# cliangyu/video-diffusion

Measured on AMD Instinct MI355X. Metric: denoise-steps/sec, higher is better.
Workload: dtype f32

## Files before the change

include/vd_amd.h:

```cpp
#ifndef VD_AMD_H
#define VD_AMD_H
#ifdef __cplusplus
extern "C" {
#endif

typedef struct vd_config {
    int image_size;
    int num_channels;
    int num_res_blocks;
    int num_heads;
    int T;
    int n_attention_ds;
    int attention_ds[8];
    int use_scale_shift_norm;
    int use_spatial_encoding;
    int use_frame_encoding;
    int enforce_position_invariance;
    int use_rpe_net;
    int allow_interactions_between_padding;
    float rp_alpha, rp_beta, rp_gamma;
    int time_embed_mult;
    int cond_emb_type;
    int learn_sigma;
} vd_config;
// ... 119 lines not shown
int vd_profile_classes(void);
const char* vd_profile_class_name(int i);

int vd_math_mode(void);
long long vd_split_image_u16(long long n_out, long long k_total);

int vd_op_conv(const float* src0, const float* src1, int C0, int Cin, int nfr, int Hs, int Ws, int ups, int stride,
               int pad, int ksz, const float* w_packed, const float* w_frag, const float* w_wino, const float* bias,
               const float* affA, const float* affB, int act, const float* res, const float* fbias, int fbias_ld,
               float* out, int Cout, void* stream);
int vd_conv_stats_split(int Hout);
int vd_conv_wino_block_couts(int nfr, int H, int Cin, int Cout);
int vd_op_conv_stats(const float* src0, int Cin, int nfr, int Hs, int Ws, int ups, const float* w_wino, const float* bias,
                     const float* res, const float* fbias, int fbias_ld, float* out, int Cout, double* gn_part,
                     void* stream);
int vd_op_gn_affine(const double* part0, int split0, int C0, const double* part1, int split1, int C, int nfr, int HW,
                    const float* gamma, const float* beta, const float* film, int film_ld, float* affA, float* affB,
                    void* stream);
int vd_pack_conv3_wino(const float* host_oihw, float* host_out, int O, int I);
int vd_pack_linear_frag(const float* host_w, float* host_out, int N, int K);
int vd_pack_linear_split(const float* host_w, unsigned short* host_out, int N, int K);
int vd_pack_conv3_split(const float* host_oihw, unsigned short* host_out, int O, int I);
int vd_op_conv_split(const float* src0, int Cin, int nfr, int Hs, int Ws, int stride, const void* w_split, const float* bias,
                     const float* res, float* out, int Cout, void* stream);
int vd_pack_conv3_wino_split(const float* host_oihw, unsigned short* host_out, int O, int I);
int vd_op_conv_wino_split(const float* src0, int Cin, int nfr, int Hs, int Ws, int ups, const void* w_split, const float* bias,
                          const float* res, const float* fbias, int fbias_ld, float* out, int Cout, double* gn_part,
                          void* stream);
int vd_op_conv_wino_act(const float* src0, const float* src1, int C0, int Cin, int nfr, int Hs, int Ws, const void* w_split, const float* bias,
                        const float* affA, const float* affB, const float* res, float* out, int Cout, double* gn_part, void* stream);
int vd_conv_wino_act_ok(int nfr, int H, int Cin, int Cout);
int vd_pack_conv3_wino_ups(const float* host_oihw, unsigned short* host_out, int O, int I);
int vd_conv_ups_stats_split(int Hs);
int vd_op_conv_wino_ups(const float* src0, int Cin, int nfr, int Hs, const void* w_ups, const float* bias, float* out, int Cout,
                        double* gn_part, void* stream);
int vd_op_linear_split(const float* a, int M, int K, const void* w_split, const float* bias, const float* res, int act,
                       float* out, int N, void* stream);
int vd_op_linear_split_stats(const float* a, int M, int K, const void* w_split, const float* bias, const float* res, int act,
                             float* out, int N, int HW, double* gn_part, void* stream);
int vd_linear_stats_split(int M, int N, int HW);
int vd_op_gn_fold(const float* src0, const float* src1, int C0, int C, int nfr, int HW, const float* gamma,
                  const float* beta, const float* film, int film_ld, float* affA, float* affB, void* stream);
int vd_op_affine_apply(const float* x, const float* affA, const float* affB, int nfr, int HW, int C, float* y,
                       void* stream);
int vd_op_affine_act(const float* src0, const float* src1, int C0, int C, const float* affA, const float* affB, int nfr,
                     int HW, int act, float* y, void* stream);
int vd_op_gn_temporal(const float* x, const float* gamma, const float* beta, int B, int T, int HW, int C, float* y,
                      void* stream);
int vd_op_attn_spatial(const float* qkv, int nfr, int L, int C, int heads, float* out, void* stream);
int vd_op_attn_temporal(const float* qkv, const float* Rk, const float* Rq, const float* Rv, const float* mask, int B,
                        int T, int HW, int C, int heads, int allow_pad, float* out, void* stream);
int vd_op_out_conv(const float* x, const float* affA, const float* affB, const float* w_packed, const float* bias,
                   int nfr, int H, int W, int C, int Cout, float* out_nchw, void* stream);
int vd_op_gn_bwd(const float* x0, const float* x1, int C0, int C, const float* affA, const float* affB, const float* mr,
                 const float* dy, int act, int nfr, int HW, const float* extra, float* dx0, int acc0, float* dx1, int acc1,
                 void* stream);
int vd_op_gn_temporal_bwd(const float* x, const float* gamma, const float* dy, int B, int T, int HW, int C, int accumulate,
                          float* dx, void* stream);
int vd_op_attn_temporal_bwd(const float* qkv, const float* Rk, const float* Rq, const float* Rv, const float* mask, int B,
                            int T, int HW, int C, int heads, int allow_pad, const float* dout, float* dqkv, void* stream);
int vd_op_attn_spatial_bwd(const float* qkv, int nfr, int L, int C, int heads, const float* dout, float* dqkv, void* stream);
int vd_op_out_conv_bwd(const float* deps, const float* w, int nfr, int H, int W, int C, int Cout, float* da, void* stream);
int vd_op_stem_col2im(const float* dcols, const float* obs, const float* lat, const float* km, int nfr, int H, int W,
                      int cond_mode, float* dx, void* stream);

typedef struct vd_lpips vd_lpips;
int vd_lpips_create(vd_lpips** out);
void vd_lpips_destroy(vd_lpips* h);
int vd_lpips_load_weight(vd_lpips* h, const char* name, const float* host, long long bytes);
long long vd_lpips_dim(int H, int W);
int vd_lpips_embed(vd_lpips* h, int N, int H, int W, const float* frames, float* out, void* stream);
int vd_fps_select(int B, int n_cand, long long D, const float* embs, int n, const int* always_host, int n_always, float* work,
                  int* out, void* stream);

int vd_frame_metrics(int N, int C, int H, int W, const float* gt, const void* pred, int pred_is_u8, double ssim_data_range,
                     double* ssim_out, double* psnr_out, void* stream);
int vd_pair_sqdist(int N, long long D, const float* a, const float* b, double* out, void* stream);

typedef struct vd_i3d vd_i3d;
int vd_i3d_create(vd_i3d** out);
void vd_i3d_destroy(vd_i3d* h);
int vd_i3d_load_weight(vd_i3d* h, const char* name, const float* host, long long bytes);
int vd_i3d_max_frames(void);
int vd_i3d_embed(vd_i3d* h, int N, int T, int H, int W, const unsigned char* videos, float* out, void* stream);
int vd_op_conv3d_same(const float* x, const float* w, const float* bias, int T, int H, int W, int Cin, int Cout, int kt, int kh,
                      int kw, int st, int sh, int sw, int relu, float* out, long long out_stride, void* stream);
int vd_op_maxpool3d_same(const float* x, int T, int H, int W, int C, int kt, int kh, int kw, int st, int sh, int sw, float* out,
                         void* stream);
int vd_op_resize_bilinear_tf1(const unsigned char* frames, int T, int H, int W, float* out, void* stream);

#ifdef __cplusplus
}
#endif
#endif
```

video-diffusion_amd/_lib.py:

```python
import ctypes
import os
import subprocess

_HERE = os.path.dirname(os.path.abspath(__file__))
_CSRC = os.path.join(_HERE, "csrc")
SO_PATH = os.path.join(_HERE, "libvdamd.so")
SOURCES = ["igemm.hip", "conv_wino.hip", "conv_wino_r64.hip", "conv_wino_z128.hip", "gemm_frag.hip", "gemm_split.hip", "split_pack.hip", "norm.hip", "backward.hip", "attn_spatial.hip", "attn_temporal.hip", "attn_temporal_long.hip", "misc.hip", "engine.hip", "lpips.hip", "metrics.hip", "i3d.hip"]
HEADER = os.path.join(os.path.dirname(_HERE), "include", "vd_amd.h")
HEADERS = [os.path.join(_CSRC, "vd_common.h"), os.path.join(_CSRC, "wino_common.h"), HEADER]
SOURCE_FLAGS = {"conv_wino_z128.hip": ["-mllvm", "-pragma-unroll-threshold=1000000"]}


def _toolchain():
    hipcc = os.environ.get("HIPCC", "/opt/rocm/bin/hipcc")
    flags = ["--offload-arch=gfx950", "-O3", "-std=c++17", "-fPIC", "-Wno-unused-value"] + \
        os.environ.get("VD_HIPCC_FLAGS", "").split()
    return hipcc, flags


def _sha(*parts):
    import hashlib
    h = hashlib.sha1()
    for p in parts:
        h.update(p if isinstance(p, bytes) else str(p).encode())
        h.update(b"\0")
    return h.hexdigest()


def _read(path):
    with open(path, "rb") as f:
        return f.read()


def source_sha():
    hipcc, flags = _toolchain()
    return _sha("\0".join(flags), repr(sorted(SOURCE_FLAGS.items())), *[_read(os.path.join(_CSRC, s)) for s in SOURCES], *[_read(h) for h in HEADERS])[:16]


def _stale():
    if not os.path.exists(SO_PATH):
        return True
    try:
        with open(SO_PATH + ".flags") as f:
            return f.read().strip() != source_sha()
    except OSError:
        return True


def build(force=False, verbose=False):
    if not force and not _stale():
        return SO_PATH
    import fcntl
    from concurrent.futures import ThreadPoolExecutor
    with open(SO_PATH + ".lock", "w") as lock:
        fcntl.flock(lock, fcntl.LOCK_EX)
        try:
            if not force and not _stale():
                return SO_PATH
            hipcc, flags = _toolchain()
            sha = source_sha()
            objdir = os.path.join(_CSRC, ".obj")
            os.makedirs(objdir, exist_ok=True)
# ... 90 lines not shown
    "vd_window_generation": (_U, [_P]),
    "vd_set_window_prefix_cache": (_I, [_P, _I]),
    "vd_window_prefix_frames": (_I, [_P]),
    "vd_set_window_suffix_skip": (_I, [_P, _I]),
    "vd_window_suffix_frames": (_I, [_P]),
    "vd_window_begin": (_I, [_P, _I, _I, _P, _P, _P, _P, _P, _P, _I, _I, _I, _F, _U, _U, _L, _P]),
    "vd_window_run": (_I, [_P, _I, _P]),
    "vd_window_graphs": (_I, [_P]),
    "vd_posterior_update": (_I, [_P, _I, _I, _L, _P, _P, _P, _I, _F, _P, _U, _U, _P, _P, _P]),
    "vd_posterior_from_xstart": (_I, [_P, _I, _I, _L, _P, _P, _P, _I, _F, _P, _U, _U, _P, _P, _P, _P]),
    "vd_attn_blocks": (_I, [_P]),
    "vd_attn_block_info": (_I, [_P, _I, ctypes.POINTER(_I), ctypes.POINTER(_I)]),
    "vd_set_attn_capture": (_I, [_P, _P, _P, _I]),
    "vd_bwd_weights_bytes": (_L, [_P]),
    "vd_set_bwd_weight_storage": (_I, [_P, _P, _L, _I]),
    "vd_load_weight_bwd": (_I, [_P, ctypes.c_char_p, _P, _L]),
    "vd_guided_step": (_I, [_P, _I, _I, _P, _P, _P, _P, _P, _P, _I, _P, _P, _P, _P, _P, _P, _P, _P]),
    "vd_q_sample": (_I, [_P, _I, _L, _P, _P, _P, _P, _P]),
    "vd_randn": (_I, [_P, _L, _U, _U, _P]),
    "vd_profile_begin": (_I, []),
    "vd_profile_end": (_I, [_P, _I]),
    "vd_profile_classes": (_I, []),
    "vd_profile_class_name": (ctypes.c_char_p, [_I]),
    "vd_op_conv": (_I, [_P, _P, _I, _I, _I, _I, _I, _I, _I, _I, _I, _P, _P, _P, _P, _P, _P, _I, _P, _P, _I, _P, _I, _P]),
    "vd_conv_stats_split": (_I, [_I]),
    "vd_conv_wino_block_couts": (_I, [_I, _I, _I, _I]),
    "vd_op_conv_stats": (_I, [_P, _I, _I, _I, _I, _I, _P, _P, _P, _P, _I, _P, _I, _P, _P]),
    "vd_op_gn_affine": (_I, [_P, _I, _I, _P, _I, _I, _I, _I, _P, _P, _P, _I, _P, _P, _P]),
    "vd_pack_conv3_wino": (_I, [_P, _P, _I, _I]),
    "vd_pack_linear_frag": (_I, [_P, _P, _I, _I]),
    "vd_pack_linear_split": (_I, [_P, _P, _I, _I]),
    "vd_pack_conv3_wino_split": (_I, [_P, _P, _I, _I]),
    "vd_set_model_mean_type": (_I, [_P, _I]),
    "vd_math_mode": (_I, []),
    "vd_split_image_u16": (_L, [_L, _L]),
    "vd_pack_conv3_wino_ups": (_I, [_P, _P, _I, _I]),
    "vd_conv_ups_stats_split": (_I, [_I]),
    "vd_op_conv_wino_ups": (_I, [_P, _I, _I, _I, _P, _P, _P, _I, _P, _P]),
    "vd_op_conv_wino_split": (_I, [_P, _I, _I, _I, _I, _I, _P, _P, _P, _P, _I, _P, _I, _P, _P]),
    "vd_op_conv_wino_act": (_I, [_P, _P, _I, _I, _I, _I, _I, _P, _P, _P, _P, _P, _P, _I, _P, _P]),
    "vd_conv_wino_act_ok": (_I, [_I, _I, _I, _I]),
    "vd_pack_conv3_split": (_I, [_P, _P, _I, _I]),
    "vd_op_conv_split": (_I, [_P, _I, _I, _I, _I, _I, _P, _P, _P, _P, _I, _P]),
    "vd_op_linear_split": (_I, [_P, _I, _I, _P, _P, _P, _I, _P, _I, _P]),
    "vd_op_linear_split_stats": (_I, [_P, _I, _I, _P, _P, _P, _I, _P, _I, _I, _P, _P]),
    "vd_linear_stats_split": (_I, [_I, _I, _I]),
    "vd_op_gn_fold": (_I, [_P, _P, _I, _I, _I, _I, _P, _P, _P, _I, _P, _P, _P]),
    "vd_op_affine_apply": (_I, [_P, _P, _P, _I, _I, _I, _P, _P]),
    "vd_op_affine_act": (_I, [_P, _P, _I, _I, _P, _P, _I, _I, _I, _P, _P]),
    "vd_op_gn_temporal": (_I, [_P, _P, _P, _I, _I, _I, _I, _P, _P]),
    "vd_op_attn_spatial": (_I, [_P, _I, _I, _I, _I, _P, _P]),
    "vd_op_attn_temporal": (_I, [_P, _P, _P, _P, _P, _I, _I, _I, _I, _I, _I, _P, _P]),
    "vd_op_out_conv": (_I, [_P, _P, _P, _P, _P, _I, _I, _I, _I, _I, _P, _P]),
    "vd_op_gn_bwd": (_I, [_P, _P, _I, _I, _P, _P, _P, _P, _I, _I, _I, _P, _P, _I, _P, _I, _P]),
    "vd_op_gn_temporal_bwd": (_I, [_P, _P, _P, _I, _I, _I, _I, _I, _P, _P]),
    "vd_op_attn_temporal_bwd": (_I, [_P, _P, _P, _P, _P, _I, _I, _I, _I, _I, _I, _P, _P, _P]),
    "vd_op_attn_spatial_bwd": (_I, [_P, _I, _I, _I, _I, _P, _P, _P]),
    "vd_op_out_conv_bwd": (_I, [_P, _P, _I, _I, _I, _I, _I, _P, _P]),
    "vd_op_stem_col2im": (_I, [_P, _P, _P, _P, _I, _I, _I, _I, _P, _P]),
    "vd_lpips_create": (_I, [ctypes.POINTER(_P)]),
    "vd_lpips_destroy": (None, [_P]),
    "vd_lpips_load_weight": (_I, [_P, ctypes.c_char_p, _P, _L]),
    "vd_lpips_dim": (_L, [_I, _I]),
    "vd_lpips_embed": (_I, [_P, _I, _I, _I, _P, _P, _P]),
    "vd_fps_select": (_I, [_I, _I, _L, _P, _I, _P, _I, _P, _P, _P]),
    "vd_frame_metrics": (_I, [_I, _I, _I, _I, _P, _P, _I, _D, _P, _P, _P]),
    "vd_pair_sqdist": (_I, [_I, _L, _P, _P, _P, _P]),
    "vd_i3d_create": (_I, [ctypes.POINTER(_P)]),
    "vd_i3d_destroy": (None, [_P]),
    "vd_i3d_load_weight": (_I, [_P, ctypes.c_char_p, _P, _L]),
    "vd_i3d_max_frames": (_I, []),
    "vd_i3d_embed": (_I, [_P, _I, _I, _I, _I, _P, _P, _P]),
    "vd_op_conv3d_same": (_I, [_P, _P, _P, _I, _I, _I, _I, _I, _I, _I, _I, _I, _I, _I, _I, _P, _L, _P]),
    "vd_op_maxpool3d_same": (_I, [_P, _I, _I, _I, _I, _I, _I, _I, _I, _I, _I, _P, _P]),
    "vd_op_resize_bilinear_tf1": (_I, [_P, _I, _I, _I, _P, _P]),
}

_lib = None


def lib():
    global _lib
    if _lib is None:
        path = os.environ.get("VD_LIB")
        if not path:
            build()
            path = SO_PATH
        L = ctypes.CDLL(path)
        for name, (res, args) in SIGNATURES.items():
            fn = getattr(L, name)
            fn.restype = res
            fn.argtypes = args
        if not os.environ.get("VD_LIB") and L.vd_source_sha().decode() != source_sha():
            raise RuntimeError(f"libvdamd.so was built from other sources ({L.vd_source_sha().decode()}) than the ones beside it "
                               f"({source_sha()}): rebuild (video_diffusion_amd._lib.build(force=True))")
        _lib = L
    return _lib


class VdError(RuntimeError):
    pass


def check(rc):
    if rc != 0:
        msg = lib().vd_last_error().decode(errors="replace")
# ... 15 lines not shown
```

video-diffusion_amd/csrc/engine.hip:

```cpp
#include <cmath>
#include <cstring>
#include <unordered_map>
#include <vector>

#include "../../include/vd_amd.h"
#include "vd_common.h"

namespace vd {

thread_local std::string g_last_error;
void set_error(const std::string& msg) { g_last_error = msg; }

int launch_frame_t(const int64_t* fidx, int B, int T, int center, float* tv, hipStream_t s);

enum ParamKind { PK_RAW = 0, PK_CONV3, PK_STEM, PK_POSENC, PK_OUTCONV, PK_LINF, PK_CONV3W, PK_CONV3S,
                 PK_CONV3WU };

struct Param {
    std::string name;
    int nd = 0;
    long long shape[4] = {1, 1, 1, 1};
    size_t numel = 0;
    size_t packed = 0;
    size_t off = 0;
    int kind = PK_RAW;
    bool loaded = false;
    int frag_rows = 0, frag_row0 = 0;
    int kind_bwd = -1;
    size_t off_bwd = 0, packed_bwd = 0;
};

struct ResP {
    int cin, cout;
    int gn1w, gn1b, c1w, c1b, embw, embb, gn2w, gn2b, c2w, c2b, skw = -1, skb = -1;
    int film_off = 0;
};
struct RpeP { int dw = -1, db = -1, tw = -1, tb = -1, ow = -1, ob = -1, table = -1; int te_off = 0; };
struct AttP { int normw, normb, qkvw, qkvb, projw, projb; };
struct AttnP { int C; AttP sp, tp; RpeP rq, rk, rv; };
struct ConvP { int w, b, c; };
struct Layer { int type; int idx; };
struct Tens { float* p; int C, H; double* part = nullptr; int split = 0; };

struct TapeRes { int idx; Tens x0, x1; bool has_x1; int N; float *A1, *B1, *mr1, *h, *A2, *B2, *mr2, *o; };
struct TapeAttn { int idx; Tens x; int B, T; float *xn, *qkv, *Rk, *Rq, *Rv, *o, *xt, *A, *Bf, *mr, *xn2, *qkv2, *o2, *xs; const float* amask; };
struct TapeConv { int type, idx; Tens in, out; };
struct TapePos { Tens in, out; };
struct TapeOp { int kind, i; };
struct Tape {
    std::vector<TapeOp> ops;
    std::vector<TapeRes> res; std::vector<TapeAttn> attn; std::vector<TapeConv> conv; std::vector<TapePos> pos;
    Tens head; float *headA = nullptr, *headB = nullptr, *head_mr = nullptr;
    void clear() { ops.clear(); res.clear(); attn.clear(); conv.clear(); pos.clear(); }
};

static const int CH_MULT_256[] = {1, 1, 2, 2, 4, 4};
static const int CH_MULT_128[] = {1, 1, 2, 3, 4};
static const int CH_MULT_64[] = {1, 2, 3, 4};
// ... 976 lines not shown
            hs.push_back(h);
        }
        if ((int)i + 1 == n_before_attn && (cfg.use_spatial_encoding || cfg.use_frame_encoding)) {
            const size_t n = (size_t)N * h.H * h.H * h.C;
            float* y = ar.get<float>(n);
            if (!ar.dry) {
                VD_REQUIRE(h.H == pos_res && h.C == pos_ch, "positional encoding shape");
                if ((rc = launch_posenc_add(h.p, cfg.use_spatial_encoding ? W(p_posenc) : nullptr, femb, N, h.H * h.H, h.C, y, st)))
                    return rc;
            }
            if (tape) { tape->ops.push_back(TapeOp{5, (int)tape->pos.size()}); tape->pos.push_back(TapePos{h, Tens{y, h.C, h.H}}); }
            h = Tens{y, h.C, h.H};
        }
    }
    if ((rc = run(middle, h, nullptr, &h))) return rc;
    const int Nsuf = sp ? sp->n : N;
    bool compact = false;
    auto gather_t = [&](const Tens& t) -> Tens {
        const size_t per = (size_t)t.H * t.H * t.C;
        Tens c{ar.get<float>((size_t)Nsuf * per), t.C, t.H, nullptr, t.split};
        if (t.part) c.part = ar.get<double>((size_t)Nsuf * t.split * t.C * 2);
        if (!ar.dry) {
            if (launch_gather_rows(t.p, sp->list, Nsuf, per, c.p, st)) return Tens{};
            if (t.part && launch_gather_rows(reinterpret_cast<const float*>(t.part), sp->list, Nsuf, (size_t)t.split * t.C * 4,
                                             reinterpret_cast<float*>(c.part), st)) return Tens{};
        }
        return c;
    };
    auto go_compact = [&]() -> int {
        float* fc = ar.get<float>((size_t)Nsuf * film_total);
        if (!ar.dry && (rc = launch_gather_rows(film_full, sp->list, Nsuf, film_total, fc, st))) return rc;
        h = gather_t(h);
        VD_REQUIRE(ar.dry || h.p, "suffix skip: gather");
        film = fc; Nrun = Nsuf; g_sel_nfr = N; compact = true;
        return 0;
    };
    if (sp && suf_blk < 0 && (rc = go_compact())) return rc;
    for (size_t i = 0; i < output_blocks.size(); ++i) {
        Tens skip = hs.back(); hs.pop_back();
        if (sp && !compact && (int)i == suf_blk) {
            if ((rc = run(output_blocks[i], h, &skip, &h, 0, suf_layer + 1))) return rc;
            if ((rc = go_compact())) return rc;
            if ((rc = run(output_blocks[i], h, nullptr, &h, suf_layer + 1))) return rc;
            continue;
        }
        if (compact) { skip = gather_t(skip); VD_REQUIRE(ar.dry || skip.p, "suffix skip: gather"); }
        if ((rc = run(output_blocks[i], h, &skip, &h))) return rc;
    }
    float *A, *Bf, *mrh = nullptr;
    if ((rc = gn_fold(h, nullptr, Nrun, p_outgw, p_outgb, nullptr, 0, st, ar, &A, &Bf, &mrh))) return rc;
    if (tape) { tape->head = h; tape->headA = A; tape->headB = Bf; tape->head_mr = mrh; }
    const int oc = cfg.learn_sigma ? 6 : 3;
    float* eps_c = compact ? ar.get<float>((size_t)Nsuf * oc * S * S) : nullptr;
    float* head_t = ar.get<float>((size_t)Nrun * S * S * out_t_cols(oc));
    if (!ar.dry) {
        VD_REQUIRE(h.H == S && h.C == final_ch, "output head shape");
        {
          ProfScope ps(PC_OUT_CONV, 2.0 * Nrun * S * S * h.C * 27.0, 4.0 * Nrun * S * S * (h.C + 3.0), st);
          if (head_gemm_supported(S * S, h.C, out_t_cols(oc))) {
              rc = launch_head_gemm(h.p, A, Bf, W(p_outw) + (size_t)9 * oc * h.C, Nrun, S * S, h.C, out_t_cols(oc), head_t, st);
          } else {
              IgemmArgs g = conv_args(h, nullptr, Nrun, 1, 1, 0);
              g.w = W(p_outw) + (size_t)9 * oc * h.C; g.wsplit = 0; g.affA = A; g.affB = Bf; g.act = 1;
              g.out = head_t; g.ldo = out_t_cols(oc); g.Cout = out_t_cols(oc);
              rc = launch_igemm(g, st);
          }
          if (!rc) rc = launch_out_gather(head_t, W(p_outb), Nrun, S, S, out_t_cols(oc), oc, compact ? eps_c : in.eps, st); }
        if (rc) return rc;
        if (compact) {
            VD_HIP(hipMemsetAsync(in.eps, 0, (size_t)N * oc * S * S * sizeof(float), st));
            if ((rc = launch_scatter_rows(eps_c, sp->list, Nsuf, (size_t)oc * S * S, in.eps, st))) return rc;
        }
    }
    VD_REQUIRE(!ar.overflow, "workspace overflow: the forward asked for more than the dry run measured (this step's output is invalid)");
    return 0;
}

int vd_engine::ensure_ws(int B, int T, bool suffix_plan) {
    const bool suf = suffix_skip_on || suffix_plan;
    if (B == ws_B && T == ws_T && ws && ws_suf == suf) return 0;
    const long long key = ((long long)B << 32) | (unsigned)T | (suf ? 1ll << 61 : 0);
    size_t tail = 0;
    int rc = grow_ws(key, step_tail_bytes(B, T), [&](size_t* peak) {
        Arena dry; dry.dry = true;
        FwdIn fi{}; fi.B = B; fi.T = T;
        int frc = forward(fi, nullptr, dry);
        if (!frc && suf) {
            Arena dry2; dry2.dry = true;
            SuffixPlan wp; wp.n = B * T;
            frc = forward(fi, nullptr, dry2, nullptr, &wp);
            dry.peak = std::max(dry.peak, dry2.peak);
        }
        *peak = dry.peak;
        return frc;
    }, &tail);
    if (rc) return rc;
    ws_B = B; ws_T = T; ws_tail = tail; ws_suf = suf;
    return 0;
}


namespace {
struct GradMap {
    std::unordered_map<const float*, std::pair<float*, bool>> m;
    Arena* ar;
    float* get(const Tens& t, int N, bool* fresh) {
        auto it = m.find(t.p);
        if (it == m.end()) it = m.emplace(t.p, std::make_pair(ar->get<float>((size_t)N * t.H * t.H * t.C), false)).first;
        *fresh = !it->second.second;
        it->second.second = true;
        return it->second.first;
    }
    float* have(const float* p) const { auto it = m.find(p); return it == m.end() ? nullptr : it->second.first; }
};
}

int vd_engine::bwd_linear(const float* dy, int M, int pw, const float* resid, float* out, hipStream_t st) {
    const Param& p = params[pw];
    const int Kb = (int)p.shape[0], Nb = p.kind == PK_STEM ? STEM_KPAD : (int)p.shape[1];
    IgemmArgs g = linear_args(M, Kb, Nb);
// ... 1119 lines not shown
    g.stats = gn_part; g.stats_split = conv_wino_stats_split(g.Ho);
    VD_REQUIRE(conv_wino_supported(g), "vd_op_conv_stats: shape not covered by the Winograd kernel");
    return launch_igemm(g, static_cast<hipStream_t>(stream));
}

int vd_op_gn_affine(const double* part0, int split0, int C0, const double* part1, int split1, int C, int nfr, int HW,
                    const float* gamma, const float* beta, const float* film, int film_ld, float* affA, float* affB,
                    void* stream) {
    return launch_gn_affine(part0, split0, C0, part1, split1, (double)HW * (C / 32), gamma, beta, film, film_ld, nfr, C, affA,
                            affB, static_cast<hipStream_t>(stream));
}

int vd_op_gn_fold(const float* src0, const float* src1, int C0, int C, int nfr, int HW, const float* gamma,
                  const float* beta, const float* film, int film_ld, float* affA, float* affB, void* stream) {
    OpScratch ws(stream);
    const int split = gn_stats_split(nfr, HW, C);
    double* part;
    int rc = ws.get(&part, (size_t)nfr * split * C * 2);
    if (!rc) rc = launch_gn_stats(src0, src1, C0, C, nfr, HW, part, split, ws.st);
    if (!rc) rc = launch_gn_affine(part, split, C, nullptr, 0, (double)HW * (C / 32), gamma, beta, film, film_ld, nfr, C, affA, affB, ws.st);
    return rc;
}

int vd_op_affine_act(const float* src0, const float* src1, int C0, int C, const float* affA, const float* affB, int nfr,
                     int HW, int act, float* y, void* stream) {
    return launch_affine_act(src0, src1, C0, C, affA, affB, nfr, HW, act, y, static_cast<hipStream_t>(stream));
}

int vd_op_affine_apply(const float* x, const float* affA, const float* affB, int nfr, int HW, int C, float* y, void* stream) {
    return launch_affine_apply(x, affA, affB, nfr, HW, C, y, static_cast<hipStream_t>(stream));
}

int vd_op_gn_temporal(const float* x, const float* gamma, const float* beta, int B, int T, int HW, int C, float* y,
                      void* stream) {
    return launch_gn_temporal(x, gamma, beta, B, T, HW, C, y, static_cast<hipStream_t>(stream));
}

int vd_op_attn_spatial(const float* qkv, int nfr, int L, int C, int heads, float* out, void* stream) {
    AttnSpatialArgs a{qkv, out, nfr, L, C, heads, 1.0f / sqrtf((float)(C / heads))};
    return launch_attn_spatial(a, static_cast<hipStream_t>(stream));
}

int vd_op_attn_temporal(const float* qkv, const float* Rk, const float* Rq, const float* Rv, const float* mask, int B,
                        int T, int HW, int C, int heads, int allow_pad, float* out, void* stream) {
    AttnTemporalArgs a{qkv, Rk, Rq, Rv, mask, out, B, T, HW, C, heads, allow_pad, 1.0f / sqrtf((float)(C / heads))};
    return launch_attn_temporal(a, static_cast<hipStream_t>(stream));
}

int vd_op_out_conv(const float* x, const float* affA, const float* affB, const float* w, const float* bias, int nfr,
                   int H, int W, int C, int Cout, float* out, void* stream) {
    return launch_out_conv(x, affA, affB, w, bias, nfr, H, W, C, Cout, out, static_cast<hipStream_t>(stream));
}

int vd_op_gn_bwd(const float* x0, const float* x1, int C0, int C, const float* affA, const float* affB, const float* mr,
                 const float* dy, int act, int nfr, int HW, const float* extra, float* dx0, int acc0, float* dx1, int acc1,
                 void* stream) {
    VD_REQUIRE(nfr > 0 && HW > 0 && C > 0 && C % 32 == 0 && C <= 1024, "vd_op_gn_bwd: shape");
    OpScratch ws(stream);
    double* part = nullptr;
    float* K = nullptr;
    int rc = ws.get(&part, (size_t)nfr * gn_bwd_split(nfr, HW, C) * C * 2);
    if (!rc) rc = ws.get(&K, (size_t)nfr * 32 * 2);
    if (rc) return rc;
    GnBwdArgs a{x0, x1, C0, C, affA, affB, mr, dy, act, nfr, HW, dx0, dx1, acc0, acc1, extra, part, K};
    return launch_gn_bwd(a, ws.st);
}

int vd_op_gn_temporal_bwd(const float* x, const float* gamma, const float* dy, int B, int T, int HW, int C, int accumulate,
                          float* dx, void* stream) {
    return launch_gn_temporal_bwd(x, gamma, dy, B, T, HW, C, accumulate, dx, static_cast<hipStream_t>(stream));
}

int vd_op_attn_temporal_bwd(const float* qkv, const float* Rk, const float* Rq, const float* Rv, const float* mask, int B,
                            int T, int HW, int C, int heads, int allow_pad, const float* dout, float* dqkv, void* stream) {
    AttnTemporalArgs a{qkv, Rk, Rq, Rv, mask, nullptr, B, T, HW, C, heads, allow_pad, 1.0f / sqrtf((float)(C / heads))};
    return launch_attn_temporal_bwd(a, dout, dqkv, static_cast<hipStream_t>(stream));
}

int vd_op_attn_spatial_bwd(const float* qkv, int nfr, int L, int C, int heads, const float* dout, float* dqkv, void* stream) {
    VD_REQUIRE(nfr > 0 && L > 0 && heads > 0 && C % heads == 0, "vd_op_attn_spatial_bwd: shape");
    AttnSpatialArgs a{qkv, nullptr, nfr, L, C, heads, 1.0f / sqrtf((float)(C / heads))};
    OpScratch ws(stream);
    float* buf = nullptr;
    int rc = ws.get(&buf, attn_spatial_bwd_ws_floats(a));
    return rc ? rc : launch_attn_spatial_bwd(a, dout, dqkv, buf, ws.st);
}

int vd_op_out_conv_bwd(const float* deps, const float* w, int nfr, int H, int W, int C, int Cout, float* da, void* stream) {
    return launch_out_conv_bwd(deps, w, nfr, H, W, C, Cout, da, static_cast<hipStream_t>(stream));
}

int vd_op_stem_col2im(const float* dcols, const float* obs, const float* lat, const float* km, int nfr, int H, int W,
                      int cond_mode, float* dx, void* stream) {
    return launch_stem_col2im(dcols, obs, lat, km, nfr, H, W, STEM_KPAD, cond_mode, dx, static_cast<hipStream_t>(stream));
}

}
```

video-diffusion_amd/csrc/misc.hip:

```cpp
#include <algorithm>

#include "vd_common.h"

namespace vd {

__global__ __launch_bounds__(256) void assemble_kernel(AssembleArgs a) {
    const int n = a.frame_list ? a.frame_list[blockIdx.y] : blockIdx.y;
    const int HW = a.H * a.W;
    const float om = a.obs_mask[n], lm = a.lat_mask[n], km = a.km_mask[n];
    const float any = fminf(om + lm + km, 1.0f);
    const int Cs = a.cond_mode == 0 ? 5 : (a.cond_mode == 1 ? 6 : 3);
    if (blockIdx.x == 0 && threadIdx.x == 0 && !a.frame_list) {
        const float t = a.t_model[n / a.T];
        const float tobs = a.obs_t_mode == 0 ? 0.f : (a.obs_t_mode == 1 ? t : t - 1.f);
        float tf = t;
        if (a.cond_mode == 0) tf = tobs * om + t * (1.f - om);
        else if (a.cond_mode == 2) {
            bool any_obs = false;
            for (int k = 0; k < a.T; ++k) any_obs |= a.obs_mask[(n / a.T) * a.T + k] == 1.f;
            if (any_obs) tf = -1.f;
        }
        a.t_frames[n] = tf;
        a.amask[n] = any;
    }
    if (a.scalars_only) return;
    constexpr int SW = 64;
    __shared__ float tile[3][SW + 2][6];
    __shared__ int lut[256];
    const int strips = (a.W + SW - 1) / SW;
    const int y = blockIdx.x / strips, x0 = (blockIdx.x - y * strips) * SW;
    for (int i = threadIdx.x; i < 9 * (SW + 2); i += 256) {
        const int xx = i % (SW + 2), rc = i / (SW + 2), r = rc % 3, c = rc / 3;
        const int yy = y + r - 1, gx = x0 + xx - 1;
        const bool in = yy >= 0 && yy < a.H && gx >= 0 && gx < a.W;
        float xv = 0.f, ov = 0.f;
        if (in) {
            const size_t q = ((size_t)n * 3 + c) * HW + yy * a.W + gx;
            xv = a.x[q];
            ov = a.obs_src[q];
        }
        if (a.cond_mode == 0) {
            tile[r][xx][c] = in ? xv * lm + ov * om + xv * (1.f - any) : 0.f;
            if (c == 0) { tile[r][xx][3] = in ? om : 0.f; tile[r][xx][4] = in ? km : 0.f; }
        } else if (a.cond_mode == 1) {
            tile[r][xx][c] = in ? xv * lm + xv * (1.f - any) : 0.f;
            tile[r][xx][3 + c] = in ? ov * om : 0.f;
        } else tile[r][xx][c] = xv;
    }
    for (int k = threadIdx.x; k < a.Kpad; k += 256) {
        const int tap = k / Cs, c = k - tap * Cs;
        lut[k] = k < 9 * Cs ? ((tap / 3) * (SW + 2) + tap % 3) * 6 + c : -1;
    }
    __syncthreads();
    const int qpr = a.Kpad >> 2, sh = 31 - __clz(qpr);
// ... 289 lines not shown
            }
        }
        float* dst = T + (pix0 + (size_t)it * 32 + 4 * kh) * LDT + lr;
#pragma unroll
        for (int ct = 0; ct < NCT; ++ct)
#pragma unroll
            for (int r = 0; r < 16; ++r) dst[(size_t)((r & 3) + 8 * (r >> 2)) * LDT + ct * 32] = acc[ct][r];
#pragma unroll
        for (int i = 0; i < NI; ++i) xa[i] = xn[i];
    }
}

bool head_gemm_supported(int HW, int C, int ldt) { return HW % 1024 == 0 && C % 8 == 0 && C <= 128 && ldt == 32; }

int launch_head_gemm(const float* h, const float* affA, const float* affB, const float* Wt, int nfr, int HW, int C, int ldt, float* T, hipStream_t s) {
    VD_REQUIRE(head_gemm_supported(HW, C, ldt), "output head GEMM: whole 1024-pixel blocks of a frame, C <= 128, 32 columns");
    const int tpw = (size_t)nfr * HW / 1024 < 512 ? 2 : 8;
    const dim3 grid((unsigned)((size_t)nfr * HW / (128 * tpw)));
    hipLaunchKernelGGL((head_gemm_kernel<1, 128>), grid, dim3(256), 0, s, h, affA, affB, Wt, HW, C, tpw, T);
    VD_HIP(hipGetLastError());
    return 0;
}

template <int LDT>
__global__ __launch_bounds__(256) void out_gather_kernel(const float* __restrict__ T, const float* __restrict__ bias, int H, int W, int Cout,
                                                         float* __restrict__ out) {
    constexpr int ROW = LDT + 4;
    __shared__ __attribute__((aligned(16))) float tile[(OT + 2) * (OT + 2) * ROW];
    const int n = blockIdx.z, y0 = blockIdx.y * OT, x0 = blockIdx.x * OT;
    const int tid = threadIdx.x, ty = tid / OT, tx = tid % OT;
    for (int i = tid; i < (OT + 2) * (OT + 2) * (LDT / 4); i += 256) {
        const int pix = i / (LDT / 4), q = i - pix * (LDT / 4);
        const int iy = y0 + pix / (OT + 2) - 1, ix = x0 + pix % (OT + 2) - 1;
        f32x4 v = {0.f, 0.f, 0.f, 0.f};
        if (iy >= 0 && iy < H && ix >= 0 && ix < W) v = *reinterpret_cast<const f32x4*>(T + (((size_t)n * H + iy) * W + ix) * LDT + q * 4);
        *reinterpret_cast<f32x4*>(tile + pix * ROW + q * 4) = v;
    }
    __syncthreads();
    const int oy = y0 + ty, ox = x0 + tx;
    if (oy >= H || ox >= W) return;
    for (int co = 0; co < Cout; ++co) {
        float acc = bias[co];
#pragma unroll
        for (int tap = 0; tap < 9; ++tap) acc += tile[((ty + tap / 3) * (OT + 2) + tx + tap % 3) * ROW + co * 9 + tap];
        out[(((size_t)n * Cout + co) * H + oy) * W + ox] = acc;
    }
}

int launch_out_gather(const float* T, const float* bias, int nfr, int H, int W, int ldt, int Cout, float* out_nchw, hipStream_t s) {
    VD_REQUIRE((ldt == 32 || ldt == 64) && 9 * Cout <= ldt, "output head: 3 or 6 output channels");
    const dim3 grid((W + OT - 1) / OT, (H + OT - 1) / OT, nfr);
    if (ldt == 32) hipLaunchKernelGGL(out_gather_kernel<32>, grid, dim3(256), 0, s, T, bias, H, W, Cout, out_nchw);
    else hipLaunchKernelGGL(out_gather_kernel<64>, grid, dim3(256), 0, s, T, bias, H, W, Cout, out_nchw);
    VD_HIP(hipGetLastError());
    return 0;
}

__device__ __forceinline__ void philox4x32_10(unsigned long long ctr, unsigned long long key, unsigned (&o)[4]) {
    unsigned c0 = (unsigned)ctr, c1 = (unsigned)(ctr >> 32), c2 = 0x5eed5eedu, c3 = 0;
    unsigned k0 = (unsigned)key, k1 = (unsigned)(key >> 32);
#pragma unroll
    for (int r = 0; r < 10; ++r) {
        const unsigned long long p0 = (unsigned long long)0xD2511F53u * c0;
        const unsigned long long p1 = (unsigned long long)0xCD9E8D57u * c2;
        const unsigned n0 = (unsigned)(p1 >> 32) ^ c1 ^ k0, n1 = (unsigned)p1;
        const unsigned n2 = (unsigned)(p0 >> 32) ^ c3 ^ k1, n3 = (unsigned)p0;
        c0 = n0; c1 = n1; c2 = n2; c3 = n3;
        k0 += 0x9E3779B9u; k1 += 0xBB67AE85u;
    }
    o[0] = c0; o[1] = c1; o[2] = c2; o[3] = c3;
}

__device__ __forceinline__ float normal_at(unsigned long long seed, unsigned long long offset, unsigned long long i) {
    unsigned r[4];
    philox4x32_10(offset + (i >> 2), seed, r);
    const int pair = (int)(i & 2);
    const float u1 = ((float)r[pair] + 1.0f) * 2.3283064365386963e-10f;
    const float u2 = (float)r[pair + 1] * 2.3283064365386963e-10f;
    const float rad = sqrtf(-2.0f * logf(u1));
    float sn, cs;
    sincosf(6.283185307179586f * u2, &sn, &cs);
    return (i & 1) ? rad * sn : rad * cs;
}

__global__ __launch_bounds__(256) void randn_kernel(float* out, size_t n, unsigned long long seed,
                                                    unsigned long long offset) {
    for (size_t i = (size_t)blockIdx.x * 256 + threadIdx.x; i < n; i += (size_t)gridDim.x * 256)
        out[i] = normal_at(seed, offset, i);
}

int launch_randn(float* out, long n, unsigned long long seed, unsigned long long offset, hipStream_t s) {
    const int grid = (int)std::min<long>((n + 255) / 256, 4096);
    hipLaunchKernelGGL(randn_kernel, dim3(grid), dim3(256), 0, s, out, (size_t)n, seed, offset);
    VD_HIP(hipGetLastError());
    return 0;
}

__global__ __launch_bounds__(256) void posterior_kernel(PosteriorArgs a) {
    const size_t total = (size_t)a.B * a.per;
    if (a.dstate) { a.seed = a.dstate[0]; a.offset = a.dstate[1]; }
    bool nonfinite = false;
    for (size_t i = (size_t)blockIdx.x * 256 + threadIdx.x; i < total; i += (size_t)gridDim.x * 256) {
        const int b = (int)(i / a.per);
        const long long tl = a.t[b];
        const int NT = a.num_timesteps;
        if (tl < 0 || tl >= NT) {
// ... 314 lines not shown
```

Before: 50.95.

## Fuse output-head GEMM and 3x3 gather into one banded kernel

Adds a single kernel that applies the GroupNorm affine and SiLU, computes the per-pixel 27-column tap projection with MFMA into LDS for a band of rows plus halo, then sums the 3x3 taps with bias straight into NCHW output. It is used when shapes allow (3 output channels, C up to 128) and replaces the head GEMM plus separate gather kernel. This drops the global intermediate tensor and one launch. In exchange, halo pixels are recomputed per band and occupancy is limited by the large LDS tile.

Result: no change. 50.94, median of 3 (-0.0%).

```diff
diff --git a/include/vd_amd.h b/include/vd_amd.h
--- a/include/vd_amd.h
+++ b/include/vd_amd.h
@@ -195,6 +195,10 @@
                         int T, int HW, int C, int heads, int allow_pad, float* out, void* stream);
 int vd_op_out_conv(const float* x, const float* affA, const float* affB, const float* w_packed, const float* bias,
                    int nfr, int H, int W, int C, int Cout, float* out_nchw, void* stream);
+int vd_op_head_fused(const float* x, const float* affA, const float* affB, const float* wt, const float* bias, int nfr, int H, int W,
+                     int C, int band, float* out_nchw, void* stream);
+int vd_op_head_gemm_gather(const float* x, const float* affA, const float* affB, const float* wt, const float* bias, int nfr, int H,
+                           int W, int C, float* T, float* out_nchw, void* stream);
 int vd_op_gn_bwd(const float* x0, const float* x1, int C0, int C, const float* affA, const float* affB, const float* mr,
                  const float* dy, int act, int nfr, int HW, const float* extra, float* dx0, int acc0, float* dx1, int acc1,
                  void* stream);
diff --git a/video-diffusion_amd/_lib.py b/video-diffusion_amd/_lib.py
--- a/video-diffusion_amd/_lib.py
+++ b/video-diffusion_amd/_lib.py
@@ -7,7 +7,7 @@
 SO_PATH = os.path.join(_HERE, "libvdamd.so")
 SOURCES = ["igemm.hip", "conv_wino.hip", "conv_wino_r64.hip", "conv_wino_z128.hip", "gemm_frag.hip", "gemm_split.hip", "split_pack.hip", "norm.hip", "backward.hip", "attn_spatial.hip", "attn_temporal.hip", "attn_temporal_long.hip", "misc.hip", "engine.hip", "lpips.hip", "metrics.hip", "i3d.hip"]
 HEADER = os.path.join(os.path.dirname(_HERE), "include", "vd_amd.h")
-HEADERS = [os.path.join(_CSRC, "vd_common.h"), os.path.join(_CSRC, "wino_common.h"), HEADER]
+HEADERS = [os.path.join(_CSRC, "vd_common.h"), os.path.join(_CSRC, "wino_common.h"), os.path.join(_CSRC, "fused_ops.h"), HEADER]
 SOURCE_FLAGS = {"conv_wino_z128.hip": ["-mllvm", "-pragma-unroll-threshold=1000000"]}
 
 
@@ -204,6 +204,8 @@
     "vd_op_attn_spatial": (_I, [_P, _I, _I, _I, _I, _P, _P]),
     "vd_op_attn_temporal": (_I, [_P, _P, _P, _P, _P, _I, _I, _I, _I, _I, _I, _P, _P]),
     "vd_op_out_conv": (_I, [_P, _P, _P, _P, _P, _I, _I, _I, _I, _I, _P, _P]),
+    "vd_op_head_fused": (_I, [_P, _P, _P, _P, _P, _I, _I, _I, _I, _I, _P, _P]),
+    "vd_op_head_gemm_gather": (_I, [_P, _P, _P, _P, _P, _I, _I, _I, _I, _P, _P, _P]),
     "vd_op_gn_bwd": (_I, [_P, _P, _I, _I, _P, _P, _P, _P, _I, _I, _I, _P, _P, _I, _P, _I, _P]),
     "vd_op_gn_temporal_bwd": (_I, [_P, _P, _P, _I, _I, _I, _I, _I, _P, _P]),
     "vd_op_attn_temporal_bwd": (_I, [_P, _P, _P, _P, _P, _I, _I, _I, _I, _I, _I, _P, _P, _P]),
diff --git a/video-diffusion_amd/csrc/engine.hip b/video-diffusion_amd/csrc/engine.hip
--- a/video-diffusion_amd/csrc/engine.hip
+++ b/video-diffusion_amd/csrc/engine.hip
@@ -4,6 +4,7 @@
 #include <vector>
 
 #include "../../include/vd_amd.h"
+#include "fused_ops.h"
 #include "vd_common.h"
 
 namespace vd {
@@ -1086,12 +1087,15 @@
     if (tape) { tape->head = h; tape->headA = A; tape->headB = Bf; tape->head_mr = mrh; }
     const int oc = cfg.learn_sigma ? 6 : 3;
     float* eps_c = compact ? ar.get<float>((size_t)Nsuf * oc * S * S) : nullptr;
-    float* head_t = ar.get<float>((size_t)Nrun * S * S * out_t_cols(oc));
+    const bool head_fused = head_fused_supported(S * S, final_ch, oc);
+    float* head_t = head_fused ? nullptr : ar.get<float>((size_t)Nrun * S * S * out_t_cols(oc));
     if (!ar.dry) {
         VD_REQUIRE(h.H == S && h.C == final_ch, "output head shape");
         {
           ProfScope ps(PC_OUT_CONV, 2.0 * Nrun * S * S * h.C * 27.0, 4.0 * Nrun * S * S * (h.C + 3.0), st);
-          if (head_gemm_supported(S * S, h.C, out_t_cols(oc))) {
+          if (head_fused) {
+              rc = launch_head_fused(h.p, A, Bf, W(p_outw) + (size_t)9 * oc * h.C, W(p_outb), Nrun, S, S, h.C, oc, 0, compact ? eps_c : in.eps, st);
+          } else if (head_gemm_supported(S * S, h.C, out_t_cols(oc))) {
               rc = launch_head_gemm(h.p, A, Bf, W(p_outw) + (size_t)9 * oc * h.C, Nrun, S * S, h.C, out_t_cols(oc), head_t, st);
           } else {
               IgemmArgs g = conv_args(h, nullptr, Nrun, 1, 1, 0);
@@ -1099,7 +1103,7 @@
               g.out = head_t; g.ldo = out_t_cols(oc); g.Cout = out_t_cols(oc);
               rc = launch_igemm(g, st);
           }
-          if (!rc) rc = launch_out_gather(head_t, W(p_outb), Nrun, S, S, out_t_cols(oc), oc, compact ? eps_c : in.eps, st); }
+          if (!rc && !head_fused) rc = launch_out_gather(head_t, W(p_outb), Nrun, S, S, out_t_cols(oc), oc, compact ? eps_c : in.eps, st); }
         if (rc) return rc;
         if (compact) {
             VD_HIP(hipMemsetAsync(in.eps, 0, (size_t)N * oc * S * S * sizeof(float), st));
@@ -2325,6 +2329,17 @@
     return launch_out_conv(x, affA, affB, w, bias, nfr, H, W, C, Cout, out, static_cast<hipStream_t>(stream));
 }
 
+int vd_op_head_fused(const float* x, const float* affA, const float* affB, const float* wt, const float* bias, int nfr, int H, int W, int C,
+                     int band, float* out, void* stream) {
+    return launch_head_fused(x, affA, affB, wt, bias, nfr, H, W, C, 3, band, out, static_cast<hipStream_t>(stream));
+}
+
+int vd_op_head_gemm_gather(const float* x, const float* affA, const float* affB, const float* wt, const float* bias, int nfr, int H, int W,
+                           int C, float* T, float* out, void* stream) {
+    const int rc = launch_head_gemm(x, affA, affB, wt, nfr, H * W, C, 32, T, static_cast<hipStream_t>(stream));
+    return rc ? rc : launch_out_gather(T, bias, nfr, H, W, 32, 3, out, static_cast<hipStream_t>(stream));
+}
+
 int vd_op_gn_bwd(const float* x0, const float* x1, int C0, int C, const float* affA, const float* affB, const float* mr,
                  const float* dy, int act, int nfr, int HW, const float* extra, float* dx0, int acc0, float* dx1, int acc1,
                  void* stream) {
diff --git a/video-diffusion_amd/csrc/fused_ops.h b/video-diffusion_amd/csrc/fused_ops.h
--- /dev/null
+++ b/video-diffusion_amd/csrc/fused_ops.h
@@ -0,0 +1,10 @@
+#pragma once
+#include "vd_common.h"
+
+namespace vd {
+
+bool head_fused_supported(int HW, int C, int Cout);
+int launch_head_fused(const float* h, const float* affA, const float* affB, const float* Wt, const float* bias, int nfr, int H, int W, int C, int Cout,
+                      int band, float* out_nchw, hipStream_t s);
+
+}
diff --git a/video-diffusion_amd/csrc/misc.hip b/video-diffusion_amd/csrc/misc.hip
--- a/video-diffusion_amd/csrc/misc.hip
+++ b/video-diffusion_amd/csrc/misc.hip
@@ -1,5 +1,6 @@
 #include <algorithm>
 
+#include "fused_ops.h"
 #include "vd_common.h"
 
 namespace vd {
@@ -395,6 +396,96 @@
     const dim3 grid((W + OT - 1) / OT, (H + OT - 1) / OT, nfr);
     if (ldt == 32) hipLaunchKernelGGL(out_gather_kernel<32>, grid, dim3(256), 0, s, T, bias, H, W, Cout, out_nchw);
     else hipLaunchKernelGGL(out_gather_kernel<64>, grid, dim3(256), 0, s, T, bias, H, W, Cout, out_nchw);
+    VD_HIP(hipGetLastError());
+    return 0;
+}
+
+constexpr int HF_BW = 64, HF_COLS = 27;
+template <int BR, int NWAVE, int CMAX>
+__global__ __launch_bounds__(NWAVE * 64, 8 / NWAVE) void head_fused_kernel(const float* __restrict__ h, const float* __restrict__ affA, const float* __restrict__ affB,
+                                                                const float* __restrict__ Wt, const float* __restrict__ bias, int H, int W, int C, int Cout,
+                                                                float* __restrict__ out) {
+    constexpr int NI = CMAX / 8;
+    __shared__ __attribute__((aligned(16))) float sab[2 * CMAX];
+    __shared__ float tl[(BR + 2) * (HF_BW + 2) * HF_COLS];
+    const int tid = threadIdx.x, lane = tid & 63, wv = tid >> 6, lr = lane & 31, kh = lane >> 5;
+    const int n = blockIdx.z, y0 = blockIdx.y * BR, x0 = blockIdx.x * HF_BW;
+    const int ry0 = max(y0 - 1, 0), ry1 = min(y0 + BR + 1, H), cx0 = max(x0 - 1, 0), cx1 = min(x0 + HF_BW + 1, W);
+    const int RW = cx1 - cx0, npix = RW * (ry1 - ry0), ntiles = (npix + 31) >> 5;
+    for (int c = tid; c < C; c += NWAVE * 64) { sab[c] = affA[(size_t)n * C + c]; sab[CMAX + c] = affB[(size_t)n * C + c]; }
+    const int ni = C >> 3;
+    f32x4 w[NI];
+#pragma unroll
+    for (int i = 0; i < NI; ++i)
+        w[i] = i < ni ? *reinterpret_cast<const f32x4*>(Wt + (size_t)lr * C + 8 * i + 4 * kh) : f32x4{0.f, 0.f, 0.f, 0.f};
+    __syncthreads();
+    auto row_of = [&](int tile) -> const float* {
+        const int p = min(tile * 32 + lr, npix - 1), ry = p / RW, rx = p - ry * RW;
+        return h + (((size_t)n * H + ry0 + ry) * W + cx0 + rx) * C + 4 * kh;
+    };
+    f32x4 xa[NI];
+    if (wv < ntiles) {
+        const float* src = row_of(wv);
+#pragma unroll
+        for (int i = 0; i < NI; ++i) xa[i] = i < ni ? *reinterpret_cast<const f32x4*>(src + 8 * i) : f32x4{0.f, 0.f, 0.f, 0.f};
+    }
+#pragma unroll 1
+    for (int tile = wv; tile < ntiles; tile += NWAVE) {
+        f32x4 xn[NI];
+        const float* nsrc = row_of(tile + NWAVE < ntiles ? tile + NWAVE : tile);
+#pragma unroll
+        for (int i = 0; i < NI; ++i) xn[i] = i < ni ? *reinterpret_cast<const f32x4*>(nsrc + 8 * i) : f32x4{0.f, 0.f, 0.f, 0.f};
+        f32x16 acc;
+#pragma unroll
+        for (int r = 0; r < 16; ++r) acc[r] = 0.f;
+#pragma unroll
+        for (int i = 0; i < NI; ++i) {
+            if (i < ni) {
+                const f32x4 Aq = *reinterpret_cast<const f32x4*>(sab + 8 * i + 4 * kh), Bq = *reinterpret_cast<const f32x4*>(sab + CMAX + 8 * i + 4 * kh);
+                f32x4 v = xa[i] * Aq + Bq;
+                v.x = silu_f(v.x); v.y = silu_f(v.y); v.z = silu_f(v.z); v.w = silu_f(v.w);
+#pragma unroll
+                for (int e = 0; e < 4; ++e) acc = __builtin_amdgcn_mfma_f32_32x32x2f32(v[e], w[i][e], acc, 0, 0, 0);
+            }
+        }
+        if (lr < HF_COLS) {
+#pragma unroll
+            for (int r = 0; r < 16; ++r) {
+                const int p = tile * 32 + 4 * kh + (r & 3) + 8 * (r >> 2);
+                if (p < npix) tl[p * HF_COLS + lr] = acc[r];
+            }
+        }
+#pragma unroll
+        for (int i = 0; i < NI; ++i) xa[i] = xn[i];
+    }
+    __syncthreads();
+    for (int i = tid; i < BR * HF_BW; i += NWAVE * 64) {
+        const int ty = i / HF_BW, tx = i - ty * HF_BW, oy = y0 + ty, ox = x0 + tx;
+        if (oy >= H || ox >= W) continue;
+        for (int co = 0; co < Cout; ++co) {
+            float acc = bias[co];
+#pragma unroll
+            for (int tap = 0; tap < 9; ++tap) {
+                const int yy = oy + tap / 3 - 1, xx = ox + tap % 3 - 1;
+                const bool in = yy >= 0 && yy < H && xx >= 0 && xx < W;
+                acc += in ? tl[((yy - ry0) * RW + xx - cx0) * HF_COLS + co * 9 + tap] : 0.f;
+            }
+            out[(((size_t)n * Cout + co) * H + oy) * W + ox] = acc;
+        }
+    }
+}
+
+bool head_fused_supported(int HW, int C, int Cout) { return head_gemm_supported(HW, C, 32) && 9 * Cout <= HF_COLS; }
+
+int launch_head_fused(const float* h, const float* affA, const float* affB, const float* Wt, const float* bias, int nfr, int H, int W, int C, int Cout,
+                      int band, float* out_nchw, hipStream_t s) {
+    VD_REQUIRE(head_fused_supported(H * W, C, Cout), "fused output head: the shapes of the head GEMM, 3 output channels");
+    VD_REQUIRE(band == 0 || band == 8 || band == 16, "fused output head: bands of 8 or 16 rows");
+    const int strips = (W + HF_BW - 1) / HF_BW;
+    if (!band) band = (size_t)nfr * strips * ((H + 15) / 16) >= 512 ? 16 : 8;
+    const dim3 grid(strips, (H + band - 1) / band, nfr);
+    if (band == 16) hipLaunchKernelGGL((head_fused_kernel<16, 8, 128>), grid, dim3(512), 0, s, h, affA, affB, Wt, bias, H, W, C, Cout, out_nchw);
+    else hipLaunchKernelGGL((head_fused_kernel<8, 4, 128>), grid, dim3(256), 0, s, h, affA, affB, Wt, bias, H, W, C, Cout, out_nchw);
     VD_HIP(hipGetLastError());
     return 0;
 }
```
